# aokomoriuta/ConjugateGradient

Hardware: AMD Instinct MI355X
Metric: CG iterations/sec (7-pt Poisson 512^3); SpMV achieved HBM GB/s in roofline (higher is better)
Workload: dtype f64

## Files before the change

### conjugategradient_amd/csrc/common.hpp

```cpp
#pragma once
#include <hip/hip_runtime.h>
#include <cstddef>
#include <cstdint>
#include <cstdio>
#include <cstdarg>
#include <cstring>
#include <cmath>
#include <atomic>
#include <mutex>
#include <string>
#include <type_traits>
#include <vector>

#pragma GCC visibility push(default)
#include "../../include/MgcgGpu.h"
#pragma GCC visibility pop

namespace mgcg {

constexpr int kWave = 64;
constexpr int kBlock = 256;
constexpr int kNumXcd = 8;
constexpr int kNumCu = 256;
constexpr int kMaxGrid = kNumCu * 8;
// ... 101 lines not shown
    double alphaPrev, betaPrev;
    int live[kShiftMaxK];
};
struct ShiftScalars {
    double sigma[kShiftMaxK];
    ShiftState st[2];
    double residual[kShiftMaxK];
    int iteration[kShiftMaxK], status[kShiftMaxK];
};

struct MixedScalars {
    double maxrr, fMaxrr;
    int want, fWant;
    int gate;
    int updates;
    int fBroken;
    int pad;
};

struct SreduceScalars {
    double red[3];
    struct State { double gamma, alpha; } st[2];
};

struct MinresScalars {
    double red[5];
    int fDone, pad;
    struct State { double beta, cs, sn, dbar, eps, phibar, oldb; } st[2];
};

struct BlockScalars;
struct BkScalars;
struct Workspace {
    int device = -1;
    hipStream_t stream = nullptr;
    double* partials = nullptr;
    CgScalars* scalars = nullptr;
    HostMirror* mirror = nullptr;
    double* hostScalar = nullptr;
    int* devInts = nullptr;
    double* trace = nullptr;
    int traceCap = 0;
    double* ring[kXDeferMax] = {};
    long long ringSize = 0;
    double* blockPartials = nullptr;
    BlockScalars* blockScalars = nullptr;
    ShiftScalars* shiftScalars = nullptr;
    double* gramPartials = nullptr;
    BkScalars* bkScalars = nullptr;
    MixedScalars* mixedScalars = nullptr;
    float* mixedVecs = nullptr;
    long long mixedStride = 0;
    SreduceScalars* sreduceScalars = nullptr;
    MinresScalars* minresScalars = nullptr;
    bool init();
    void destroy();
    bool ensure_trace(int cap);
    bool ensure_ring(int slots, long long n);
    void free_ring();
    bool ensure_block();
    bool ensure_shift();
    bool ensure_bkrylov();
    bool ensure_mixed(long long n);
    bool ensure_sreduce();
    bool ensure_minres();
};

}

struct MgcgBlas   { mgcg::Workspace ws; };
namespace mgcg {
struct DcsrView {
    const unsigned char* colCode;
    const unsigned char* valCode;
    const int* deltaDict;
    const double* valueDict;
    int nDelta, nValue;
    long long rowBase;
    const unsigned char* patternId;
    const int* patCount;
    const int* patDelta;
    const double* patValue;
    int nPattern, patWidth;
    const double* tileVals;
    const int* tileCols;
    const int* tileRowIds;
    const int* tileStartHost;
    const unsigned* tilePacked;
    const int2* tileHdr;
    const int* tileHdrBaseHost;
    int tileShift;
    int tileWidth;
    int nTiles;
    long long tileRows;
    const double* pbVals;
    const unsigned short* pbCols;
    const unsigned short* pbPos;
    double* pbProd;
    const unsigned* pbPiece;
    const int* pbTileStart;
    const unsigned* pbPieceOff;
    const int* pbRoundOff;
    const unsigned short* pbRowBounds;
    int pbTiles, pbBlocks;
    long long pbColumns;
};
struct DcsrMatrix {
    const double* elements = nullptr; const int* rowOffsets = nullptr; const int* columnIndeces = nullptr;
    long long rows = 0, nnz = 0, rowBase = 0;
    unsigned char* colCode = nullptr; unsigned char* valCode = nullptr;
    int* deltaDict = nullptr; double* valueDict = nullptr;
    int nDelta = 0, nValue = 0;
    unsigned char* patternId = nullptr; int* patCount = nullptr; int* patDelta = nullptr; double* patValue = nullptr;
    int nPattern = 0, patWidth = 0;
    double* tileVals = nullptr; int* tileCols = nullptr; int* tileRowIds = nullptr; int nTiles = 0; long long tileRows = 0;
    unsigned* tilePacked = nullptr; int2* tileHdr = nullptr; int tileShift = 0, tileWidth = 0;
    std::vector<int> tileStart, tileHdrBase;
    double* pbVals = nullptr; unsigned short* pbCols = nullptr; unsigned short* pbPos = nullptr; double* pbProd = nullptr; unsigned* pbPiece = nullptr;
    unsigned* pbPieceOff = nullptr; int* pbTileStart = nullptr; int* pbRoundOff = nullptr; unsigned short* pbRowBounds = nullptr;
    int pbTiles = 0, pbBlocks = 0, pbMaxRounds = 0; long long pbColumns = 0;
    unsigned long long checksum = 0;
    int trustedUses = 0;
    bool automatic = false;
    bool usable = false;
    std::atomic<bool> stale{false};
    void release();
    DcsrView view() const
    {
        DcsrView v; v.colCode = colCode; v.valCode = valCode; v.deltaDict = deltaDict; v.valueDict = valueDict; v.nDelta = nDelta; v.nValue = nValue; v.rowBase = rowBase;
        v.patternId = patternId; v.patCount = patCount; v.patDelta = patDelta; v.patValue = patValue; v.nPattern = nPattern; v.patWidth = patWidth;
        v.tileVals = tileVals; v.tileCols = tileCols; v.tileRowIds = tileRowIds; v.tileStartHost = tileStart.data(); v.nTiles = nTiles; v.tileRows = tileRows;
        v.tilePacked = tilePacked; v.tileHdr = tileHdr; v.tileHdrBaseHost = tileHdrBase.data(); v.tileShift = tileShift; v.tileWidth = tileWidth;
        v.pbVals = pbVals; v.pbCols = pbCols; v.pbPos = pbPos; v.pbProd = pbProd; v.pbPiece = pbPiece; v.pbTileStart = pbTileStart; v.pbRoundOff = pbRoundOff;
        v.pbPieceOff = pbPieceOff; v.pbRowBounds = pbRowBounds; v.pbTiles = pbTiles; v.pbBlocks = pbBlocks; v.pbColumns = pbColumns;
        return v;
    }
};
struct SpmvProfile {
    bool enabled = false;
    std::vector<hipEvent_t> start, stop;
    int used = 0;
};
}
struct MgcgSparse {
    mgcg::Workspace ws;
    mgcg::SpmvProfile prof;
    int kernel = 0;
    int rowsPerBlock = 64;
    int flags = 0;
    int gridBlocks = 0;
    int periodRows = 0;
    int tileRows = 0, tilePlanes = 0;
    int analysedMode = 0;
    int compression = 0;
    std::vector<mgcg::DcsrMatrix*> analysed;
    struct PeriodEntry { const int* rowOffsets; const int* columnIndeces; long long rows, rowBase; int period; int maxRow; long long meanDistance;
                         int products = 0, threshold = 8; };
    std::vector<PeriodEntry> periods;
};
struct MgcgMatDescr { int type = 0; int base = 0; };
struct Vector    { double* data = nullptr; long long size = 0; int device = -1;
                   bool rawExported = false;
                   bool placed = false;
                   int drawCount = 0, drawChosen = -1; float drawMs[16] = {}; };
struct VectorInt { int* data = nullptr;    long long size = 0; int device = -1; };

namespace mgcg {

enum SpmvEpilogue {
    EPI_AXPBY = 0,
    EPI_DOT = 1,
    EPI_RESIDUAL = 2,
    EPI_JACOBI = 3,
    EPI_RESIDUAL_DOT = 4,
    EPI_AXPBY_BETA = 5,
    EPI_JACOBI_DOT = 6,
    EPI_CHEBYSHEV = 7,
    EPI_CHEBYSHEV_DOT = 8
};
#ifdef MGCG_LAB
#define MGCG_ABLATE(a, bits) (((a).ablate & (bits)) != 0)
#else
#define MGCG_ABLATE(a, bits) false
#endif
constexpr bool epi_has_dot(int e) { return e == EPI_DOT || e == EPI_RESIDUAL_DOT || e == EPI_JACOBI_DOT || e == EPI_CHEBYSHEV_DOT; }
constexpr bool epi_is_jacobi(int e) { return e == EPI_JACOBI || e == EPI_JACOBI_DOT; }
constexpr bool epi_is_chebyshev(int e) { return e == EPI_CHEBYSHEV || e == EPI_CHEBYSHEV_DOT; }

struct SpmvArgs {
    const double* elements;
    const int* rowOffsets;
    const int* columnIndeces;
    const double* x;
    double* y;
    int elementsCount;
    int rowCount;
    int columnCount;
    double alpha, beta;
    const double* w;
    const double* b;
    const double* dinv;
    double omega;
    int dinvUniform;
    double dinvScalar;
    double* d;
    double c1, c2;
    int xScaled;
    double xInner, xOuter;
    const double* xCoarse;
    int cM0, cM1, cM2, cS1, cS2;
    int cRowBase;
    double* partials;
    const int* doneFlag;
// ... 262 lines not shown
```

### conjugategradient_amd/csrc/kernels_dcsr.hip

```cpp
#include "common.hpp"
#include <algorithm>
#include <climits>

namespace mgcg {

typedef double d2 __attribute__((ext_vector_type(2)));
typedef unsigned u2 __attribute__((ext_vector_type(2)));

constexpr int kHashCap = 1024;
constexpr int kDictMax = 256;
constexpr int kEmptyDelta = INT_MIN;
constexpr unsigned long long kEmptyValue = 0xFFF8DEADBEEF0001ull;

__device__ inline void set_insert_delta(int* set, int* count, int key)
{
    unsigned h = ((unsigned)key * 2654435761u) & (kHashCap - 1);
    for (int probe = 0; probe < kHashCap; ++probe) {
        const int cur = set[h];
        if (cur == key) return;
        if (cur == kEmptyDelta) {
            const int prev = atomicCAS(&set[h], kEmptyDelta, key);
            if (prev == kEmptyDelta) { atomicAdd(count, 1); return; }
            if (prev == key) return;
        }
// ... 70 lines not shown
    h ^= h >> 33;
    return h;
}

__global__ __launch_bounds__(kBlock) void pattern_hash_kernel(const double* __restrict__ elements, const int* __restrict__ rowOffsets,
                                                              const int* __restrict__ columnIndeces, long long rows, long long rowBase,
                                                              unsigned long long* __restrict__ rowHash, unsigned long long* set, int* stats)
{
    const long long stride = (long long)gridDim.x * kBlock;
    int longest = 0;
    for (long long i = (long long)blockIdx.x * kBlock + threadIdx.x; i < rows; i += stride) {
        if (stats[0] > kPatMax) break;
        const int s = rowOffsets[i], e = rowOffsets[i + 1];
        unsigned long long h = pat_mix(0x243F6A8885A308D3ull, (unsigned long long)(e - s));
        for (int k = s; k < e; ++k) {
            h = pat_mix(h, (unsigned long long)((long long)columnIndeces[k] - (rowBase + i)));
            h = pat_mix(h, (unsigned long long)__double_as_longlong(elements[k]));
        }
        if (h == kPatEmpty) h = 1ull;
        rowHash[i] = h;
        longest = (e - s) > longest ? (e - s) : longest;
        unsigned slot = (unsigned)(h >> 20) & (kPatHashCap - 1);
        for (int probe = 0; probe < kPatHashCap; ++probe) {
            const unsigned long long cur = set[slot];
            if (cur == h) break;
            if (cur == kPatEmpty) {
                const unsigned long long prev = atomicCAS(&set[slot], kPatEmpty, h);
                if (prev == kPatEmpty) { atomicAdd(&stats[0], 1); break; }
                if (prev == h) break;
            }
            slot = (slot + 1) & (kPatHashCap - 1);
        }
    }
    atomicMax(&stats[1], longest);
}

__global__ __launch_bounds__(kBlock) void pattern_assign_kernel(const unsigned long long* __restrict__ rowHash, long long rows,
                                                                const unsigned long long* __restrict__ sorted, int n,
                                                                unsigned char* __restrict__ patternId, long long* rep)
{
    const long long stride = (long long)gridDim.x * kBlock;
    for (long long i = (long long)blockIdx.x * kBlock + threadIdx.x; i < rows; i += stride) {
        const int id = find_sorted(sorted, n, rowHash[i]);
        patternId[i] = (unsigned char)id;
        if (rep[id] > i) atomicMin((unsigned long long*)&rep[id], (unsigned long long)i);
    }
}

__global__ void pattern_table_kernel(const double* __restrict__ elements, const int* __restrict__ rowOffsets, const int* __restrict__ columnIndeces,
                                     long long rowBase, const long long* __restrict__ rep, int n, int width,
                                     int* __restrict__ patCount, int* __restrict__ patDelta, double* __restrict__ patValue)
{
    const int id = blockIdx.x * blockDim.x + threadIdx.x;
    if (id >= n) return;
    const long long i = rep[id];
    const int s = rowOffsets[i], e = rowOffsets[i + 1];
    patCount[id] = e - s;
    for (int j = 0; j < width; ++j) {
        const bool in = s + j < e;
        patDelta[id * width + j] = in ? (int)((long long)columnIndeces[s + j] - (rowBase + i)) : 0;
        patValue[id * width + j] = in ? elements[s + j] : 0.0;
    }
}

__global__ __launch_bounds__(kBlock) void pattern_verify_kernel(const double* __restrict__ elements, const int* __restrict__ rowOffsets,
                                                                const int* __restrict__ columnIndeces, long long rows, long long rowBase,
                                                                const unsigned char* __restrict__ patternId, int width,
                                                                const int* __restrict__ patCount, const int* __restrict__ patDelta,
                                                                const double* __restrict__ patValue, int* err)
{
    const long long stride = (long long)gridDim.x * kBlock;
    bool bad = false;
    for (long long i = (long long)blockIdx.x * kBlock + threadIdx.x; i < rows; i += stride) {
        const int id = patternId[i];
        const int s = rowOffsets[i], e = rowOffsets[i + 1];
        if (e - s != patCount[id]) { bad = true; continue; }
        for (int k = s; k < e; ++k) {
            const int d = (int)((long long)columnIndeces[k] - (rowBase + i));
            bad = bad || d != patDelta[id * width + (k - s)] ||
                  __double_as_longlong(elements[k]) != __double_as_longlong(patValue[id * width + (k - s)]);
        }
    }
    if (bad) atomicExch(err, 1);
}

void DcsrMatrix::release()
{
    if (colCode) (void)hipFree(colCode);
    if (valCode) (void)hipFree(valCode);
    if (deltaDict) (void)hipFree(deltaDict);
    if (valueDict) (void)hipFree(valueDict);
    if (patternId) (void)hipFree(patternId);
    if (patCount) (void)hipFree(patCount);
    if (patDelta) (void)hipFree(patDelta);
    if (patValue) (void)hipFree(patValue);
    if (tileVals) (void)hipFree(tileVals);
    if (tileCols) (void)hipFree(tileCols);
    if (tileRowIds) (void)hipFree(tileRowIds);
    if (tilePacked) (void)hipFree(tilePacked);
    if (tileHdr) (void)hipFree(tileHdr);
    tileVals = nullptr; tileCols = nullptr; tileRowIds = nullptr; nTiles = 0; tileRows = 0; tileStart.clear();
    tilePacked = nullptr; tileHdr = nullptr; tileShift = 0; tileWidth = 0; tileHdrBase.clear(); checksum = 0;
    for (void* p : { (void*)pbVals, (void*)pbCols, (void*)pbPos, (void*)pbProd, (void*)pbPiece, (void*)pbTileStart, (void*)pbPieceOff, (void*)pbRoundOff, (void*)pbRowBounds })
        if (p) (void)hipFree(p);
    pbVals = nullptr; pbCols = nullptr; pbPos = nullptr; pbProd = nullptr; pbPiece = nullptr; pbTileStart = nullptr; pbRoundOff = nullptr; pbPieceOff = nullptr;
    pbRowBounds = nullptr; pbTiles = pbBlocks = pbMaxRounds = 0; pbColumns = 0;
    colCode = valCode = nullptr; deltaDict = nullptr; valueDict = nullptr; nDelta = nValue = 0;
    patternId = nullptr; patCount = nullptr; patDelta = nullptr; patValue = nullptr; nPattern = patWidth = 0;
    usable = false;
}

bool pattern_build(hipStream_t s, const double* elements, const int* rowOffsets, const int* columnIndeces,
                   long long rows, long long nnz, long long rowBase, DcsrMatrix* out)
{
    if (rows <= 0 || nnz <= 0) return true;
    unsigned long long *rowHash = nullptr, *set = nullptr, *dSorted = nullptr;
    long long* rep = nullptr;
    int* stats = nullptr;
    unsigned char* ids = nullptr; int* pc = nullptr; int* pd = nullptr; double* pv = nullptr;
    auto cleanup = [&](bool keep) {
        for (void* p : { (void*)rowHash, (void*)set, (void*)dSorted, (void*)rep, (void*)stats }) if (p) (void)hipFree(p);
        if (!keep) for (void* p : { (void*)ids, (void*)pc, (void*)pd, (void*)pv }) if (p) (void)hipFree(p);
    };
    bool ok = MGCG_HIP(hipMalloc((void**)&rowHash, sizeof(unsigned long long) * (size_t)rows)) &&
              MGCG_HIP(hipMalloc((void**)&set, sizeof(unsigned long long) * kPatHashCap)) && MGCG_HIP(hipMalloc((void**)&stats, 3 * sizeof(int)));
    ok = ok && MGCG_HIP(hipMemsetAsync(set, 0, sizeof(unsigned long long) * kPatHashCap, s)) && MGCG_HIP(hipMemsetAsync(stats, 0, 3 * sizeof(int), s));
    if (!ok) { cleanup(false); return false; }
    long long blocks = (rows + kBlock - 1) / kBlock;
    if (blocks > kMaxGrid) blocks = kMaxGrid;
    hipLaunchKernelGGL(pattern_hash_kernel, dim3((int)blocks), dim3(kBlock), 0, s, elements, rowOffsets, columnIndeces, rows, rowBase, rowHash, set, stats);
    int hS[3] = { 0, 0, 0 };
    std::vector<unsigned long long> hSet(kPatHashCap);
    ok = MGCG_HIP(hipMemcpyAsync(hS, stats, sizeof(hS), hipMemcpyDeviceToHost, s)) &&
         MGCG_HIP(hipMemcpyAsync(hSet.data(), set, sizeof(unsigned long long) * kPatHashCap, hipMemcpyDeviceToHost, s)) && MGCG_HIP(hipStreamSynchronize(s));
    if (!ok) { cleanup(false); return false; }
    const int n = hS[0], width = hS[1];
    if (n < 1 || n > kPatMax || width < 1 || (long long)n * width > kPatEntries) { cleanup(false); return true; }
    std::vector<unsigned long long> sorted;
    for (unsigned long long v : hSet) if (v != kPatEmpty) sorted.push_back(v);
    std::sort(sorted.begin(), sorted.end());
    if ((int)sorted.size() != n) { cleanup(false); return true; }
    std::vector<long long> hRep((size_t)n, 0x7fffffffffffffffLL);
    ok = MGCG_HIP(hipMalloc((void**)&dSorted, sizeof(unsigned long long) * (size_t)n)) && MGCG_HIP(hipMalloc((void**)&rep, sizeof(long long) * (size_t)n)) &&
         MGCG_HIP(hipMalloc((void**)&ids, (size_t)rows + 16)) && MGCG_HIP(hipMalloc((void**)&pc, sizeof(int) * (size_t)n)) &&
         MGCG_HIP(hipMalloc((void**)&pd, sizeof(int) * (size_t)n * width)) && MGCG_HIP(hipMalloc((void**)&pv, sizeof(double) * (size_t)n * width));
    ok = ok && MGCG_HIP(hipMemcpyAsync(dSorted, sorted.data(), sizeof(unsigned long long) * (size_t)n, hipMemcpyHostToDevice, s)) &&
         MGCG_HIP(hipMemcpyAsync(rep, hRep.data(), sizeof(long long) * (size_t)n, hipMemcpyHostToDevice, s));
    if (!ok) { cleanup(false); return false; }
    hipLaunchKernelGGL(pattern_assign_kernel, dim3((int)blocks), dim3(kBlock), 0, s, rowHash, rows, dSorted, n, ids, rep);
    hipLaunchKernelGGL(pattern_table_kernel, dim3((n + 63) / 64), dim3(64), 0, s, elements, rowOffsets, columnIndeces, rowBase, rep, n, width, pc, pd, pv);
    hipLaunchKernelGGL(pattern_verify_kernel, dim3((int)blocks), dim3(kBlock), 0, s, elements, rowOffsets, columnIndeces, rows, rowBase, ids, width, pc, pd, pv, &stats[2]);
    ok = MGCG_HIP(hipGetLastError()) && MGCG_HIP(hipMemcpyAsync(hS, stats, sizeof(hS), hipMemcpyDeviceToHost, s)) && MGCG_HIP(hipStreamSynchronize(s));
    if (!ok) { cleanup(false); return false; }
    if (hS[2] != 0) { cleanup(false); return true; }
    out->patternId = ids; out->patCount = pc; out->patDelta = pd; out->patValue = pv; out->nPattern = n; out->patWidth = width;
    cleanup(true);
    return true;
}

bool dcsr_build(hipStream_t s, const double* elements, const int* rowOffsets, const int* columnIndeces,
                long long rows, long long nnz, long long rowBase, DcsrMatrix* out)
{
    out->release();
    out->elements = elements; out->rowOffsets = rowOffsets; out->columnIndeces = columnIndeces; out->rows = rows; out->nnz = nnz; out->rowBase = rowBase;
    if (rows <= 0 || nnz < 8) return true;
    int* dSet = nullptr; unsigned long long* vSet = nullptr; int* counts = nullptr;
    bool ok = MGCG_HIP(hipMalloc((void**)&dSet, sizeof(int) * kHashCap)) && MGCG_HIP(hipMalloc((void**)&vSet, sizeof(unsigned long long) * kHashCap)) &&
              MGCG_HIP(hipMalloc((void**)&counts, 2 * sizeof(int)));
    std::vector<int> hD(kHashCap, kEmptyDelta);
    std::vector<unsigned long long> hV(kHashCap, kEmptyValue);
    int hC[2] = { 0, 0 };
    ok = ok && MGCG_HIP(hipMemcpyAsync(dSet, hD.data(), sizeof(int) * kHashCap, hipMemcpyHostToDevice, s));
    ok = ok && MGCG_HIP(hipMemcpyAsync(vSet, hV.data(), sizeof(unsigned long long) * kHashCap, hipMemcpyHostToDevice, s));
    ok = ok && MGCG_HIP(hipMemcpyAsync(counts, hC, sizeof(hC), hipMemcpyHostToDevice, s));
    if (ok) {
        long long blocks = (rows + kBlock - 1) / kBlock;
        if (blocks > kMaxGrid) blocks = kMaxGrid;
        hipLaunchKernelGGL(dcsr_collect_kernel, dim3((int)blocks), dim3(kBlock), 0, s, elements, rowOffsets, columnIndeces, rows, rowBase, dSet, vSet, counts);
        ok = MGCG_HIP(hipMemcpyAsync(hC, counts, sizeof(hC), hipMemcpyDeviceToHost, s));
        ok = ok && MGCG_HIP(hipMemcpyAsync(hD.data(), dSet, sizeof(int) * kHashCap, hipMemcpyDeviceToHost, s));
        ok = ok && MGCG_HIP(hipMemcpyAsync(hV.data(), vSet, sizeof(unsigned long long) * kHashCap, hipMemcpyDeviceToHost, s));
        ok = ok && MGCG_HIP(hipStreamSynchronize(s));
    }
    if (dSet) (void)hipFree(dSet);
    if (vSet) (void)hipFree(vSet);
    if (counts) (void)hipFree(counts);
    if (!ok) return false;
    if (hC[0] > kDictMax) return true;
    std::vector<int> deltas;
    for (int v : hD) if (v != kEmptyDelta) deltas.push_back(v);
    std::sort(deltas.begin(), deltas.end());
    std::vector<unsigned long long> values;
    const bool val8 = hC[1] <= kDictMax;
    if (val8) { for (unsigned long long v : hV) if (v != kEmptyValue) values.push_back(v); std::sort(values.begin(), values.end()); }
    if ((int)deltas.size() != hC[0] || (val8 && (int)values.size() != hC[1])) { set_error("dcsr_build: inconsistent dictionary"); return false; }

    unsigned long long* dValBits = nullptr;
    ok = MGCG_HIP(hipMalloc((void**)&out->deltaDict, sizeof(int) * kDictMax)) && MGCG_HIP(hipMalloc((void**)&out->colCode, (size_t)nnz + 16));
    ok = ok && MGCG_HIP(hipMemcpyAsync(out->deltaDict, deltas.data(), sizeof(int) * deltas.size(), hipMemcpyHostToDevice, s));
    if (val8) {
        ok = ok && MGCG_HIP(hipMalloc((void**)&out->valueDict, sizeof(double) * kDictMax)) && MGCG_HIP(hipMalloc((void**)&out->valCode, (size_t)nnz + 16));
        ok = ok && MGCG_HIP(hipMalloc((void**)&dValBits, sizeof(unsigned long long) * kDictMax));
        ok = ok && MGCG_HIP(hipMemcpyAsync(dValBits, values.data(), sizeof(unsigned long long) * values.size(), hipMemcpyHostToDevice, s));
        ok = ok && MGCG_HIP(hipMemcpyAsync(out->valueDict, values.data(), sizeof(double) * values.size(), hipMemcpyHostToDevice, s));
    }
    if (ok) {
        long long blocks = (rows + kBlock - 1) / kBlock;
        if (blocks > kMaxGrid) blocks = kMaxGrid;
        hipLaunchKernelGGL(dcsr_encode_kernel, dim3((int)blocks), dim3(kBlock), 0, s, elements, rowOffsets, columnIndeces, rows, rowBase,
                           out->deltaDict, (int)deltas.size(), dValBits, (int)values.size(), out->colCode, val8 ? out->valCode : nullptr);
        ok = MGCG_HIP(hipGetLastError()) && MGCG_HIP(hipStreamSynchronize(s));
    }
    if (dValBits) (void)hipFree(dValBits);
    if (!ok) { out->release(); return false; }
    out->nDelta = (int)deltas.size(); out->nValue = (int)values.size(); out->usable = true;
    return true;
}

void preload_kernels_dcsr() { preload_code_object(reinterpret_cast<const void*>(&dcsr_collect_kernel)); }

}
```

### conjugategradient_amd/csrc/kernels_rows.hip

```cpp
#include "common.hpp"
#include "spmv_epilogue.hpp"

namespace mgcg {

typedef double d2 __attribute__((ext_vector_type(2)));
typedef int i2 __attribute__((ext_vector_type(2)));
typedef unsigned u2 __attribute__((ext_vector_type(2)));

enum { FMT_CSR = 0, FMT_DCSR8 = 1, FMT_DCSR64 = 2 };

constexpr int kRR = 64;
constexpr int kRCap = 512;
constexpr int kRAlign = 32;
constexpr int kRDict = 256;

template <int FMT>
struct RowsStage {
    i2 col[4];
    d2 val[4];
    u2 cc, vc;
    int my_s, my_e;
    int s, e;
};

// ... 108 lines not shown
            __syncthreads();
            double acc = 0.0;
            int k = cur.my_s;
            const int passEnd0 = tb0 + kRCap;
            double xg[8], vv[8];
            int cnt = cur.my_e - k; cnt = cnt < 8 ? cnt : 8;
            { const int room = passEnd0 - k; cnt = cnt < room ? cnt : room; cnt = cnt > 0 ? cnt : 0; }
#pragma unroll
            for (int j = 0; j < 8; ++j) {
                int idx = k + j - tb0;
                idx = (j < cnt) ? idx : 0;
                long long col;
                if constexpr (FMT == FMT_CSR) { col = s_col[idx]; vv[j] = s_val[idx]; }
                else {
                    col = myRowGlobal + s_dD[s_cc[idx]];
                    if constexpr (FMT == FMT_DCSR8) vv[j] = s_vD[s_vc[idx]]; else vv[j] = s_val[idx];
                }
                if (j >= cnt) col = 0;
                if (MGCG_ABLATE(a, 2)) col &= 1023;
                xg[j] = a.x[col];
            }
            long long myRow = r0 + tid;
            myRow = myRow <= lastRow ? myRow : lastRow;
            const RowsEpi eo = rows_epi_prefetch<EPI>(a, myRow);
            issue(nxt, t + 1 < nTrips ? rb_of(t + 1) : rb);
            if (pendRow >= 0 && !MGCG_ABLATE(a, 1)) a.y[pendRow] = pendVal;
#pragma unroll
            for (int j = 0; j < 8; ++j) { const double p = vv[j] * xg[j]; acc += (j < cnt) ? p : 0.0; }
            k += cnt;
            int tb = tb0;
            while (true) {
                const int passEnd = tb + kRCap;
                const int stop = cur.my_e < passEnd ? cur.my_e : passEnd;
                for (; k < stop; ++k) {
                    const int idx = k - tb;
                    long long col; double v;
                    if constexpr (FMT == FMT_CSR) { col = s_col[idx]; v = s_val[idx]; }
                    else { col = myRowGlobal + s_dD[s_cc[idx]]; if constexpr (FMT == FMT_DCSR8) v = s_vD[s_vc[idx]]; else v = s_val[idx]; }
                    const double p = v * a.x[col];
                    acc += p;
                }
                tb += kRCap;
                if (tb >= e) break;
                __syncthreads();
                RowsStage<FMT> more;
                more.s = cur.s; more.e = cur.e; more.my_s = cur.my_s; more.my_e = cur.my_e;
                load_pass(more, tb);
                stage_pass(more, tb, e);
                __syncthreads();
            }
            pendRow = -1;
            if (tid < nr) { pendVal = rows_epilogue_value<EPI>(a, acc, eo, dotacc); pendRow = r0 + tid; }
            if (MGCG_ABLATE(a, 1) && acc == 1.2345e300) pendRow = 0;
            __syncthreads();
            cur = nxt;
            nxt.s = s2; nxt.e = e2;
        }
        if (pendRow >= 0 && !MGCG_ABLATE(a, 1)) a.y[pendRow] = pendVal;
    }
    if constexpr (epi_has_dot(EPI)) {
        double v = dotacc;
#pragma unroll
        for (int off = 32; off > 0; off >>= 1) v += __shfl_down(v, off, 64);
        if (tid == 0) a.partials[blockIdx.x] = v;
    }
}

template <int EPI>
static int launch_rows_epi(hipStream_t s, const SpmvArgs& a, const DcsrView* m, int gridReq)
{
    const int nRowBlocks = (int)(((long long)a.rowCount + kRR - 1) / kRR);
    DeviceState* d = device_state();
    int grid = gridReq > 0 ? gridReq : (m == nullptr ? 8 : 16) * (d ? d->numCu : kNumCu);
    if (grid > kMaxPartials) grid = kMaxPartials;
    if (grid > nRowBlocks) grid = nRowBlocks;
    if (grid < 1) grid = 1;
    DcsrView none{};
    if (m == nullptr) hipLaunchKernelGGL((spmv_rows_kernel<EPI, FMT_CSR>), dim3(grid), dim3(64), 0, s, a, none, nRowBlocks);
    else if (m->valCode != nullptr) hipLaunchKernelGGL((spmv_rows_kernel<EPI, FMT_DCSR8>), dim3(grid), dim3(64), 0, s, a, *m, nRowBlocks);
    else hipLaunchKernelGGL((spmv_rows_kernel<EPI, FMT_DCSR64>), dim3(grid), dim3(64), 0, s, a, *m, nRowBlocks);
    return grid;
}

template <int EPI, int CH>
__global__ __launch_bounds__(64) void spmv_pattern_kernel(SpmvArgs a, DcsrView m, int nRowBlocks, int groupBlocks, TileMap tm)
{
    constexpr int RPL = 2;
    extern __shared__ __attribute__((aligned(16))) unsigned char s_raw[];
    const int W = m.patWidth, nP = m.nPattern;
    double* s_val = (double*)s_raw;
    int* s_delta = (int*)(s_val + nP * W);
    int* s_cnt = s_delta + nP * W;
    if (a.doneFlag != nullptr && *a.doneFlag != 0) return;
    const int tid = threadIdx.x;
    for (int i = tid; i < nP * W; i += 64) { s_val[i] = m.patValue[i]; s_delta[i] = m.patDelta[i]; }
    for (int i = tid; i < nP; i += 64) s_cnt[i] = m.patCount[i];
    __syncthreads();

    const bool grouped = groupBlocks > 0 && (gridDim.x & 7) == 0;
    const long long G = grouped ? groupBlocks : 1;
    const int xcd = grouped ? (int)(blockIdx.x & 7) : 0;
    const long long first = grouped ? (long long)(blockIdx.x >> 3) : (long long)blockIdx.x;
    const long long step = grouped ? (long long)(gridDim.x >> 3) : (long long)gridDim.x;
    const long long count = grouped ? (((long long)nRowBlocks + 8 * G - 1) / (8 * G)) * G : (long long)nRowBlocks;
    auto block_of = [&](long long L) -> long long { return grouped ? ((L / G) * 8 + xcd) * G + (L % G) : L; };

    const long long lastRow = (long long)a.rowCount - 1;
    auto load_ids = [&](long long rb, int* pid) {
        const long long base = rb * (64 * RPL);
#pragma unroll
        for (int u = 0; u < RPL; ++u) { long long r = base + u * 64 + tid; r = r <= lastRow ? r : lastRow; r = r >= 0 ? r : 0; pid[u] = m.patternId[r]; }
    };
    const bool sweep = tm.mode != 0;
    const long long nTrips = sweep ? tile_map_trips(tm, (int)blockIdx.x, (int)gridDim.x, nRowBlocks) : (count > first ? (count - first + step - 1) / step : 0);
    auto trip_block = [&](long long t) -> long long { return sweep ? (long long)tile_map_tile(tm, (int)t, (int)blockIdx.x, (int)gridDim.x) : block_of(first + t * step); };
    double dotacc = 0.0;
    int pidNext[RPL];
    if (nTrips > 0) load_ids(trip_block(0) < nRowBlocks ? trip_block(0) : 0, pidNext);
    for (long long t = 0; t < nTrips; ++t) {
        const long long rb = trip_block(t);
        int pid[RPL];
#pragma unroll
        for (int u = 0; u < RPL; ++u) pid[u] = pidNext[u];
        if (t + 1 < nTrips) { const long long nb = trip_block(t + 1); load_ids(nb < nRowBlocks ? nb : 0, pidNext); }
        if (rb >= nRowBlocks) continue;
        const long long base = rb * (64 * RPL);
        long long row[RPL]; bool live[RPL]; int tb[RPL], cnt[RPL]; double acc[RPL]; RowsEpi eo[RPL];
#pragma unroll
        for (int u = 0; u < RPL; ++u) {
            row[u] = base + u * 64 + tid;
            live[u] = row[u] <= lastRow;
            row[u] = live[u] ? row[u] : lastRow;
        }
#pragma unroll
        for (int u = 0; u < RPL; ++u) { eo[u] = rows_epi_prefetch<EPI>(a, row[u]); tb[u] = pid[u] * W; cnt[u] = s_cnt[pid[u]]; acc[u] = 0.0; }
        int longest = 0, shortest = 0x7fffffff;
#pragma unroll
        for (int u = 0; u < RPL; ++u) { longest = cnt[u] > longest ? cnt[u] : longest; shortest = cnt[u] < shortest ? cnt[u] : shortest; }
#pragma unroll
        for (int off = 32; off > 0; off >>= 1) {
            const int o = __shfl_xor(longest, off, 64), q = __shfl_xor(shortest, off, 64);
            longest = o > longest ? o : longest; shortest = q < shortest ? q : shortest;
        }
        if (shortest == CH && longest == CH) {
            double xg[RPL][CH], vv[RPL][CH];
#pragma unroll
            for (int u = 0; u < RPL; ++u) {
                const long long g = m.rowBase + row[u];
#pragma unroll
                for (int j = 0; j < CH; ++j) {
                    vv[u][j] = s_val[tb[u] + j];
                    long long col = g + s_delta[tb[u] + j];
                    if (MGCG_ABLATE(a, 2)) col &= 1023;
                    xg[u][j] = a.x[col];
                }
            }
            if (a.xScaled) {
#pragma unroll
                for (int u = 0; u < RPL; ++u)
#pragma unroll
                    for (int j = 0; j < CH; ++j) { const double t = a.xInner * xg[u][j]; xg[u][j] = a.xOuter * t; }
            }
#pragma unroll
            for (int u = 0; u < RPL; ++u)
#pragma unroll
                for (int j = 0; j < CH; ++j) { const double p = vv[u][j] * xg[u][j]; acc[u] += p; }
        } else {
            for (int j0 = 0; j0 < longest; j0 += CH) {
                double xg[RPL][CH], vv[RPL][CH];
#pragma unroll
                for (int u = 0; u < RPL; ++u) {
                    const long long g = m.rowBase + row[u];
#pragma unroll
                    for (int j = 0; j < CH; ++j) {
                        const bool on = j0 + j < cnt[u];
                        const int t = tb[u] + (on ? j0 + j : 0);
                        vv[u][j] = s_val[t];
                        xg[u][j] = a.x[g + s_delta[t]];
                    }
                }
                if (a.xScaled) {
#pragma unroll
                    for (int u = 0; u < RPL; ++u)
#pragma unroll
                        for (int j = 0; j < CH; ++j) { const double t = a.xInner * xg[u][j]; xg[u][j] = a.xOuter * t; }
                }
#pragma unroll
                for (int u = 0; u < RPL; ++u)
#pragma unroll
                    for (int j = 0; j < CH; ++j) { const double p = vv[u][j] * xg[u][j]; acc[u] += (j0 + j < cnt[u]) ? p : 0.0; }
            }
        }
#pragma unroll
        for (int u = 0; u < RPL; ++u)
            if (live[u]) {
                const double v = rows_epilogue_value<EPI>(a, acc[u], eo[u], dotacc);
                if (!MGCG_ABLATE(a, 1) || v == 1.2345e300) a.y[row[u]] = v;
            }
    }
    if constexpr (epi_has_dot(EPI)) {
        double v = dotacc;
#pragma unroll
        for (int off = 32; off > 0; off >>= 1) v += __shfl_down(v, off, 64);
        if (tid == 0) a.partials[blockIdx.x] = v;
    }
}

constexpr int kPatternWavesPerCu = 16;

template <int EPI>
static int launch_pattern_epi(hipStream_t s, const SpmvArgs& a, const DcsrView& m, int gridReq, int periodRows)
{
    const int nRowBlocks = (int)(((long long)a.rowCount + 127) / 128);
    DeviceState* d = device_state();
    int grid = gridReq > 0 ? gridReq : kPatternWavesPerCu * (d ? d->numCu : kNumCu);
    if (grid > kMaxPartials) grid = kMaxPartials;
    if (grid > nRowBlocks) grid = nRowBlocks;
    if (grid < 1) grid = 1;
    const size_t lds = (size_t)m.nPattern * m.patWidth * 12 + (size_t)m.nPattern * 4;
    const int group = 0;
    TileMap tm = make_tile_map(a.rowCount, (a.rowCount % 128 != 0) ? 0 : periodRows, grid, 128);
    if (m.patWidth == 7) hipLaunchKernelGGL((spmv_pattern_kernel<EPI, 7>), dim3(grid), dim3(64), lds, s, a, m, nRowBlocks, group, tm);
    else if (m.patWidth == 5) hipLaunchKernelGGL((spmv_pattern_kernel<EPI, 5>), dim3(grid), dim3(64), lds, s, a, m, nRowBlocks, group, tm);
    else hipLaunchKernelGGL((spmv_pattern_kernel<EPI, 8>), dim3(grid), dim3(64), lds, s, a, m, nRowBlocks, group, tm);
    return grid;
}

static int launch_spmv_pattern(hipStream_t s, int epilogue, const SpmvArgs& a, const DcsrView& m, int gridReq, int periodRows)
{
    switch (epilogue) {
    case EPI_AXPBY:        return a.beta != 0.0 ? launch_pattern_epi<EPI_AXPBY_BETA>(s, a, m, gridReq, periodRows) : launch_pattern_epi<EPI_AXPBY>(s, a, m, gridReq, periodRows);
    case EPI_DOT:          return launch_pattern_epi<EPI_DOT>(s, a, m, gridReq, periodRows);
    case EPI_RESIDUAL:     return launch_pattern_epi<EPI_RESIDUAL>(s, a, m, gridReq, periodRows);
    case EPI_RESIDUAL_DOT: return launch_pattern_epi<EPI_RESIDUAL_DOT>(s, a, m, gridReq, periodRows);
    case EPI_JACOBI:       return launch_pattern_epi<EPI_JACOBI>(s, a, m, gridReq, periodRows);
    case EPI_JACOBI_DOT:   return launch_pattern_epi<EPI_JACOBI_DOT>(s, a, m, gridReq, periodRows);
    }
    return 0;
}

int launch_spmv_rows(hipStream_t s, int epilogue, const SpmvArgs& a, const DcsrView* m, int gridReq, int periodRows)
{
    if (a.rowCount <= 0) return 0;
    if (m != nullptr && m->patternId != nullptr) return launch_spmv_pattern(s, epilogue, a, *m, gridReq, periodRows);
    switch (epilogue) {
    case EPI_AXPBY:        return a.beta != 0.0 ? launch_rows_epi<EPI_AXPBY_BETA>(s, a, m, gridReq) : launch_rows_epi<EPI_AXPBY>(s, a, m, gridReq);
    case EPI_DOT:          return launch_rows_epi<EPI_DOT>(s, a, m, gridReq);
    case EPI_RESIDUAL:     return launch_rows_epi<EPI_RESIDUAL>(s, a, m, gridReq);
    case EPI_RESIDUAL_DOT: return launch_rows_epi<EPI_RESIDUAL_DOT>(s, a, m, gridReq);
    case EPI_JACOBI:       return launch_rows_epi<EPI_JACOBI>(s, a, m, gridReq);
    case EPI_JACOBI_DOT:   return launch_rows_epi<EPI_JACOBI_DOT>(s, a, m, gridReq);
    case EPI_CHEBYSHEV:    return launch_rows_epi<EPI_CHEBYSHEV>(s, a, m, gridReq);
    case EPI_CHEBYSHEV_DOT: return launch_rows_epi<EPI_CHEBYSHEV_DOT>(s, a, m, gridReq);
    }
    return 0;
}

void preload_kernels_rows() { preload_code_object(reinterpret_cast<const void*>(&(spmv_rows_kernel<EPI_DOT, FMT_CSR>))); }

}
```

Measured before the change: 270.4.

## Add dominant-pattern fast path with wave-uniform stencil loads in pattern SpMV

Setup now builds a histogram of row pattern IDs and records the dominant full-width pattern as a reference. The SpMV kernel holds that pattern's coefficients and offsets in scalar registers and, for rows using it, loads x through a scalar base plus a lane offset, avoiding per-lane LDS lookups and 64-bit address arithmetic. Other rows take a per-lane general path. The kernel also changes from 64-thread blocks handling two rows per lane to 256-thread workgroups of four waves, one row per lane, with a different tile map and grid sizing. This trades per-row indirection for more divergence when patterns are mixed, plus extra histogram work at setup.

```diff
diff --git a/conjugategradient_amd/csrc/common.hpp b/conjugategradient_amd/csrc/common.hpp
--- a/conjugategradient_amd/csrc/common.hpp
+++ b/conjugategradient_amd/csrc/common.hpp
@@ -207,6 +207,7 @@
     const int* patDelta;
     const double* patValue;
     int nPattern, patWidth;
+    int refPattern;
     const double* tileVals;
     const int* tileCols;
     const int* tileRowIds;
@@ -237,7 +238,7 @@
     int* deltaDict = nullptr; double* valueDict = nullptr;
     int nDelta = 0, nValue = 0;
     unsigned char* patternId = nullptr; int* patCount = nullptr; int* patDelta = nullptr; double* patValue = nullptr;
-    int nPattern = 0, patWidth = 0;
+    int nPattern = 0, patWidth = 0, refPattern = -1;
     double* tileVals = nullptr; int* tileCols = nullptr; int* tileRowIds = nullptr; int nTiles = 0; long long tileRows = 0;
     unsigned* tilePacked = nullptr; int2* tileHdr = nullptr; int tileShift = 0, tileWidth = 0;
     std::vector<int> tileStart, tileHdrBase;
@@ -253,7 +254,7 @@
     DcsrView view() const
     {
         DcsrView v; v.colCode = colCode; v.valCode = valCode; v.deltaDict = deltaDict; v.valueDict = valueDict; v.nDelta = nDelta; v.nValue = nValue; v.rowBase = rowBase;
-        v.patternId = patternId; v.patCount = patCount; v.patDelta = patDelta; v.patValue = patValue; v.nPattern = nPattern; v.patWidth = patWidth;
+        v.patternId = patternId; v.patCount = patCount; v.patDelta = patDelta; v.patValue = patValue; v.nPattern = nPattern; v.patWidth = patWidth; v.refPattern = refPattern;
         v.tileVals = tileVals; v.tileCols = tileCols; v.tileRowIds = tileRowIds; v.tileStartHost = tileStart.data(); v.nTiles = nTiles; v.tileRows = tileRows;
         v.tilePacked = tilePacked; v.tileHdr = tileHdr; v.tileHdrBaseHost = tileHdrBase.data(); v.tileShift = tileShift; v.tileWidth = tileWidth;
         v.pbVals = pbVals; v.pbCols = pbCols; v.pbPos = pbPos; v.pbProd = pbProd; v.pbPiece = pbPiece; v.pbTileStart = pbTileStart; v.pbRoundOff = pbRoundOff;
diff --git a/conjugategradient_amd/csrc/kernels_dcsr.hip b/conjugategradient_amd/csrc/kernels_dcsr.hip
--- a/conjugategradient_amd/csrc/kernels_dcsr.hip
+++ b/conjugategradient_amd/csrc/kernels_dcsr.hip
@@ -176,6 +176,26 @@
         }
     }
     if (bad) atomicExch(err, 1);
+}
+
+__global__ __launch_bounds__(kBlock) void pattern_histogram_kernel(const unsigned char* __restrict__ patternId, long long rows, unsigned long long* hist)
+{
+    __shared__ unsigned int s_hist[kPatMax];
+    for (int i = threadIdx.x; i < kPatMax; i += kBlock) s_hist[i] = 0u;
+    __syncthreads();
+    const long long stride = (long long)gridDim.x * kBlock;
+    for (long long i = (long long)blockIdx.x * kBlock + threadIdx.x; i < rows; i += stride) atomicAdd(&s_hist[patternId[i]], 1u);
+    __syncthreads();
+    for (int i = threadIdx.x; i < kPatMax; i += kBlock)
+        if (s_hist[i] != 0u) atomicAdd(&hist[i], (unsigned long long)s_hist[i]);
+}
+
+__global__ void pattern_dominant_kernel(const unsigned long long* __restrict__ hist, int n, int width, const int* __restrict__ patCount, int* ref)
+{
+    if (blockIdx.x != 0 || threadIdx.x != 0) return;
+    int best = 0;
+    for (int id = 1; id < n; ++id) if (hist[id] > hist[best]) best = id;
+    *ref = patCount[best] == width ? best : -1;
 }
 
 void DcsrMatrix::release()
@@ -200,7 +220,7 @@
     pbVals = nullptr; pbCols = nullptr; pbPos = nullptr; pbProd = nullptr; pbPiece = nullptr; pbTileStart = nullptr; pbRoundOff = nullptr; pbPieceOff = nullptr;
     pbRowBounds = nullptr; pbTiles = pbBlocks = pbMaxRounds = 0; pbColumns = 0;
     colCode = valCode = nullptr; deltaDict = nullptr; valueDict = nullptr; nDelta = nValue = 0;
-    patternId = nullptr; patCount = nullptr; patDelta = nullptr; patValue = nullptr; nPattern = patWidth = 0;
+    patternId = nullptr; patCount = nullptr; patDelta = nullptr; patValue = nullptr; nPattern = patWidth = 0; refPattern = -1;
     usable = false;
 }
 
@@ -208,12 +228,12 @@
                    long long rows, long long nnz, long long rowBase, DcsrMatrix* out)
 {
     if (rows <= 0 || nnz <= 0) return true;
-    unsigned long long *rowHash = nullptr, *set = nullptr, *dSorted = nullptr;
+    unsigned long long *rowHash = nullptr, *set = nullptr, *dSorted = nullptr, *hist = nullptr;
     long long* rep = nullptr;
     int* stats = nullptr;
     unsigned char* ids = nullptr; int* pc = nullptr; int* pd = nullptr; double* pv = nullptr;
     auto cleanup = [&](bool keep) {
-        for (void* p : { (void*)rowHash, (void*)set, (void*)dSorted, (void*)rep, (void*)stats }) if (p) (void)hipFree(p);
+        for (void* p : { (void*)rowHash, (void*)set, (void*)dSorted, (void*)hist, (void*)rep, (void*)stats }) if (p) (void)hipFree(p);
         if (!keep) for (void* p : { (void*)ids, (void*)pc, (void*)pd, (void*)pv }) if (p) (void)hipFree(p);
     };
     bool ok = MGCG_HIP(hipMalloc((void**)&rowHash, sizeof(unsigned long long) * (size_t)rows)) &&
@@ -247,6 +267,15 @@
     ok = MGCG_HIP(hipGetLastError()) && MGCG_HIP(hipMemcpyAsync(hS, stats, sizeof(hS), hipMemcpyDeviceToHost, s)) && MGCG_HIP(hipStreamSynchronize(s));
     if (!ok) { cleanup(false); return false; }
     if (hS[2] != 0) { cleanup(false); return true; }
+    int ref = -1;
+    ok = MGCG_HIP(hipMalloc((void**)&hist, sizeof(unsigned long long) * kPatMax)) && MGCG_HIP(hipMemsetAsync(hist, 0, sizeof(unsigned long long) * kPatMax, s));
+    if (ok) {
+        hipLaunchKernelGGL(pattern_histogram_kernel, dim3((int)blocks), dim3(kBlock), 0, s, ids, rows, hist);
+        hipLaunchKernelGGL(pattern_dominant_kernel, dim3(1), dim3(64), 0, s, hist, n, width, pc, &stats[0]);
+        ok = MGCG_HIP(hipGetLastError()) && MGCG_HIP(hipMemcpyAsync(&ref, &stats[0], sizeof(int), hipMemcpyDeviceToHost, s)) && MGCG_HIP(hipStreamSynchronize(s));
+    }
+    if (!ok) { cleanup(false); return false; }
+    out->refPattern = (ref >= 0 && ref < n) ? ref : -1;
     out->patternId = ids; out->patCount = pc; out->patDelta = pd; out->patValue = pv; out->nPattern = n; out->patWidth = width;
     cleanup(true);
     return true;
diff --git a/conjugategradient_amd/csrc/kernels_rows.hip b/conjugategradient_amd/csrc/kernels_rows.hip
--- a/conjugategradient_amd/csrc/kernels_rows.hip
+++ b/conjugategradient_amd/csrc/kernels_rows.hip
@@ -214,148 +214,158 @@
     return grid;
 }
 
+constexpr int kPW = 4;
+constexpr int kPTileRows = 64 * kPW;
+constexpr int kPatternWgPerCu = 2;
+constexpr int kPatternTripTiles = 1;
+constexpr bool kPatternNtStore = false;
+
+__device__ __forceinline__ double pattern_uniform(double v)
+{
+    const int lo = __builtin_amdgcn_readfirstlane(__double2loint(v)), hi = __builtin_amdgcn_readfirstlane(__double2hiint(v));
+    return __hiloint2double(hi, lo);
+}
+
+typedef const __attribute__((address_space(1))) char* pattern_gptr;
+
 template <int EPI, int CH>
-__global__ __launch_bounds__(64) void spmv_pattern_kernel(SpmvArgs a, DcsrView m, int nRowBlocks, int groupBlocks, TileMap tm)
-{
-    constexpr int RPL = 2;
+__global__ __launch_bounds__(64 * kPW) void spmv_pattern_kernel(SpmvArgs a, DcsrView m, int nRowBlocks, int nTiles, TileMap tm)
+{
+    constexpr int U = kPatternTripTiles;
     extern __shared__ __attribute__((aligned(16))) unsigned char s_raw[];
     const int W = m.patWidth, nP = m.nPattern;
     double* s_val = (double*)s_raw;
     int* s_delta = (int*)(s_val + nP * W);
     int* s_cnt = s_delta + nP * W;
     if (a.doneFlag != nullptr && *a.doneFlag != 0) return;
-    const int tid = threadIdx.x;
-    for (int i = tid; i < nP * W; i += 64) { s_val[i] = m.patValue[i]; s_delta[i] = m.patDelta[i]; }
-    for (int i = tid; i < nP; i += 64) s_cnt[i] = m.patCount[i];
+    const int tid = threadIdx.x & 63;
+    const int wv = __builtin_amdgcn_readfirstlane((int)(threadIdx.x >> 6));
+    for (int i = threadIdx.x; i < nP * W; i += 64 * kPW) { s_val[i] = m.patValue[i]; s_delta[i] = m.patDelta[i]; }
+    for (int i = threadIdx.x; i < nP; i += 64 * kPW) s_cnt[i] = m.patCount[i];
     __syncthreads();
 
-    const bool grouped = groupBlocks > 0 && (gridDim.x & 7) == 0;
-    const long long G = grouped ? groupBlocks : 1;
-    const int xcd = grouped ? (int)(blockIdx.x & 7) : 0;
-    const long long first = grouped ? (long long)(blockIdx.x >> 3) : (long long)blockIdx.x;
-    const long long step = grouped ? (long long)(gridDim.x >> 3) : (long long)gridDim.x;
-    const long long count = grouped ? (((long long)nRowBlocks + 8 * G - 1) / (8 * G)) * G : (long long)nRowBlocks;
-    auto block_of = [&](long long L) -> long long { return grouped ? ((L / G) * 8 + xcd) * G + (L % G) : L; };
+    const int ref = W <= CH ? m.refPattern : -1;
+    const int nF = W;
+    double rv[CH]; int rd[CH];
+#pragma unroll
+    for (int j = 0; j < CH; ++j) {
+        const int e = (ref >= 0 && j < nF) ? ref * W + j : 0;
+        rv[j] = pattern_uniform(s_val[e]);
+        rd[j] = __builtin_amdgcn_readfirstlane(s_delta[e]);
+    }
 
     const long long lastRow = (long long)a.rowCount - 1;
-    auto load_ids = [&](long long rb, int* pid) {
-        const long long base = rb * (64 * RPL);
-#pragma unroll
-        for (int u = 0; u < RPL; ++u) { long long r = base + u * 64 + tid; r = r <= lastRow ? r : lastRow; r = r >= 0 ? r : 0; pid[u] = m.patternId[r]; }
-    };
-    const bool sweep = tm.mode != 0;
-    const long long nTrips = sweep ? tile_map_trips(tm, (int)blockIdx.x, (int)gridDim.x, nRowBlocks) : (count > first ? (count - first + step - 1) / step : 0);
-    auto trip_block = [&](long long t) -> long long { return sweep ? (long long)tile_map_tile(tm, (int)t, (int)blockIdx.x, (int)gridDim.x) : block_of(first + t * step); };
+    const int wg = blockIdx.x, nWG = gridDim.x;
+    const int nTrips = tile_map_trips(tm, wg, nWG, nTiles);
+    auto block_of = [&](int t) -> long long { return (long long)tile_map_tile(tm, t, wg, nWG) * kPW + wv; };
+    auto load_id = [&](long long rb) -> int { long long r = rb * 64 + tid; r = r <= lastRow ? r : lastRow; return m.patternId[r]; };
     double dotacc = 0.0;
-    int pidNext[RPL];
-    if (nTrips > 0) load_ids(trip_block(0) < nRowBlocks ? trip_block(0) : 0, pidNext);
-    for (long long t = 0; t < nTrips; ++t) {
-        const long long rb = trip_block(t);
-        int pid[RPL];
-#pragma unroll
-        for (int u = 0; u < RPL; ++u) pid[u] = pidNext[u];
-        if (t + 1 < nTrips) { const long long nb = trip_block(t + 1); load_ids(nb < nRowBlocks ? nb : 0, pidNext); }
-        if (rb >= nRowBlocks) continue;
-        const long long base = rb * (64 * RPL);
-        long long row[RPL]; bool live[RPL]; int tb[RPL], cnt[RPL]; double acc[RPL]; RowsEpi eo[RPL];
-#pragma unroll
-        for (int u = 0; u < RPL; ++u) {
-            row[u] = base + u * 64 + tid;
-            live[u] = row[u] <= lastRow;
-            row[u] = live[u] ? row[u] : lastRow;
-        }
-#pragma unroll
-        for (int u = 0; u < RPL; ++u) { eo[u] = rows_epi_prefetch<EPI>(a, row[u]); tb[u] = pid[u] * W; cnt[u] = s_cnt[pid[u]]; acc[u] = 0.0; }
-        int longest = 0, shortest = 0x7fffffff;
-#pragma unroll
-        for (int u = 0; u < RPL; ++u) { longest = cnt[u] > longest ? cnt[u] : longest; shortest = cnt[u] < shortest ? cnt[u] : shortest; }
-#pragma unroll
-        for (int off = 32; off > 0; off >>= 1) {
-            const int o = __shfl_xor(longest, off, 64), q = __shfl_xor(shortest, off, 64);
-            longest = o > longest ? o : longest; shortest = q < shortest ? q : shortest;
-        }
-        if (shortest == CH && longest == CH) {
-            double xg[RPL][CH], vv[RPL][CH];
-#pragma unroll
-            for (int u = 0; u < RPL; ++u) {
+    int pidNext[U];
+#pragma unroll
+    for (int u = 0; u < U; ++u) pidNext[u] = u < nTrips ? load_id(block_of(u)) : 0;
+    for (int t0 = 0; t0 < nTrips; t0 += U) {
+        int pid[U]; long long rb[U]; bool on[U];
+#pragma unroll
+        for (int u = 0; u < U; ++u) {
+            pid[u] = pidNext[u];
+            on[u] = t0 + u < nTrips;
+            rb[u] = on[u] ? block_of(t0 + u) : 0;
+            on[u] = on[u] && rb[u] < nRowBlocks;
+        }
+#pragma unroll
+        for (int u = 0; u < U; ++u)
+            if (t0 + U + u < nTrips) pidNext[u] = load_id(block_of(t0 + U + u));
+        long long row[U]; bool live[U], fastLane[U]; double acc[U]; RowsEpi eo[U]; double xg[U][CH];
+#pragma unroll
+        for (int u = 0; u < U; ++u) {
+            row[u] = rb[u] * 64 + tid;
+            live[u] = on[u] && row[u] <= lastRow;
+            row[u] = row[u] <= lastRow ? row[u] : lastRow;
+            fastLane[u] = live[u] && pid[u] == ref;
+            eo[u] = rows_epi_prefetch<EPI>(a, row[u]);
+            acc[u] = 0.0;
+        }
+#pragma unroll
+        for (int u = 0; u < U; ++u)
+            if (fastLane[u]) {
+                const double* xb = a.x + (m.rowBase + rb[u] * 64);
+                unsigned lane8 = (unsigned)tid << 3;
+                asm volatile("" : "+v"(lane8));
+#pragma unroll
+                for (int j = 0; j < CH; ++j)
+                    if (CH != 8 || j < nF) {
+                        pattern_gptr sb = (pattern_gptr)(MGCG_ABLATE(a, 2) ? a.x + j : xb + rd[j]);
+                        asm volatile("" : "+s"(sb));
+                        xg[u][j] = *(const __attribute__((address_space(1))) double*)(sb + lane8);
+                    }
+            }
+#pragma unroll
+        for (int u = 0; u < U; ++u)
+            if (live[u] && !fastLane[u]) {
                 const long long g = m.rowBase + row[u];
-#pragma unroll
-                for (int j = 0; j < CH; ++j) {
-                    vv[u][j] = s_val[tb[u] + j];
-                    long long col = g + s_delta[tb[u] + j];
-                    if (MGCG_ABLATE(a, 2)) col &= 1023;
-                    xg[u][j] = a.x[col];
-                }
-            }
-            if (a.xScaled) {
-#pragma unroll
-                for (int u = 0; u < RPL; ++u)
-#pragma unroll
-                    for (int j = 0; j < CH; ++j) { const double t = a.xInner * xg[u][j]; xg[u][j] = a.xOuter * t; }
-            }
-#pragma unroll
-            for (int u = 0; u < RPL; ++u)
-#pragma unroll
-                for (int j = 0; j < CH; ++j) { const double p = vv[u][j] * xg[u][j]; acc[u] += p; }
-        } else {
-            for (int j0 = 0; j0 < longest; j0 += CH) {
-                double xg[RPL][CH], vv[RPL][CH];
-#pragma unroll
-                for (int u = 0; u < RPL; ++u) {
-                    const long long g = m.rowBase + row[u];
+                const int tb = pid[u] * W, cnt = s_cnt[pid[u]];
+                for (int j0 = 0; j0 < cnt; j0 += CH) {
+                    double xo[CH], vv[CH];
 #pragma unroll
                     for (int j = 0; j < CH; ++j) {
-                        const bool on = j0 + j < cnt[u];
-                        const int t = tb[u] + (on ? j0 + j : 0);
-                        vv[u][j] = s_val[t];
-                        xg[u][j] = a.x[g + s_delta[t]];
+                        const bool in = j0 + j < cnt;
+                        const int t = tb + (in ? j0 + j : 0);
+                        vv[j] = s_val[t];
+                        xo[j] = a.x[g + s_delta[t]];
                     }
-                }
+                    if (a.xScaled) {
+#pragma unroll
+                        for (int j = 0; j < CH; ++j) { const double t = a.xInner * xo[j]; xo[j] = a.xOuter * t; }
+                    }
+#pragma unroll
+                    for (int j = 0; j < CH; ++j) { const double p = vv[j] * xo[j]; acc[u] += (j0 + j < cnt) ? p : 0.0; }
+                }
+            }
+#pragma unroll
+        for (int u = 0; u < U; ++u)
+            if (fastLane[u]) {
                 if (a.xScaled) {
 #pragma unroll
-                    for (int u = 0; u < RPL; ++u)
-#pragma unroll
-                        for (int j = 0; j < CH; ++j) { const double t = a.xInner * xg[u][j]; xg[u][j] = a.xOuter * t; }
-                }
-#pragma unroll
-                for (int u = 0; u < RPL; ++u)
-#pragma unroll
-                    for (int j = 0; j < CH; ++j) { const double p = vv[u][j] * xg[u][j]; acc[u] += (j0 + j < cnt[u]) ? p : 0.0; }
-            }
-        }
-#pragma unroll
-        for (int u = 0; u < RPL; ++u)
+                    for (int j = 0; j < CH; ++j)
+                        if (CH != 8 || j < nF) { const double t = a.xInner * xg[u][j]; xg[u][j] = a.xOuter * t; }
+                }
+#pragma unroll
+                for (int j = 0; j < CH; ++j)
+                    if (CH != 8 || j < nF) { const double p = rv[j] * xg[u][j]; acc[u] += p; }
+            }
+#pragma unroll
+        for (int u = 0; u < U; ++u)
             if (live[u]) {
                 const double v = rows_epilogue_value<EPI>(a, acc[u], eo[u], dotacc);
-                if (!MGCG_ABLATE(a, 1) || v == 1.2345e300) a.y[row[u]] = v;
+                if (!MGCG_ABLATE(a, 1) || v == 1.2345e300) {
+                    if constexpr (kPatternNtStore) __builtin_nontemporal_store(v, a.y + row[u]); else a.y[row[u]] = v;
+                }
             }
     }
     if constexpr (epi_has_dot(EPI)) {
         double v = dotacc;
 #pragma unroll
         for (int off = 32; off > 0; off >>= 1) v += __shfl_down(v, off, 64);
-        if (tid == 0) a.partials[blockIdx.x] = v;
-    }
-}
-
-constexpr int kPatternWavesPerCu = 16;
+        if (tid == 0) a.partials[blockIdx.x * kPW + wv] = v;
+    }
+}
 
 template <int EPI>
 static int launch_pattern_epi(hipStream_t s, const SpmvArgs& a, const DcsrView& m, int gridReq, int periodRows)
 {
-    const int nRowBlocks = (int)(((long long)a.rowCount + 127) / 128);
+    const int nRowBlocks = (int)(((long long)a.rowCount + 63) / 64);
+    const int nTiles = (int)(((long long)a.rowCount + kPTileRows - 1) / kPTileRows);
     DeviceState* d = device_state();
-    int grid = gridReq > 0 ? gridReq : kPatternWavesPerCu * (d ? d->numCu : kNumCu);
-    if (grid > kMaxPartials) grid = kMaxPartials;
-    if (grid > nRowBlocks) grid = nRowBlocks;
-    if (grid < 1) grid = 1;
+    int nWG = gridReq > 0 ? gridReq / kPW : kPatternWgPerCu * (d ? d->numCu : kNumCu);
+    if (nWG * kPW > kMaxPartials) nWG = kMaxPartials / kPW;
+    if (nWG > nTiles) nWG = nTiles;
+    if (nWG < 1) nWG = 1;
     const size_t lds = (size_t)m.nPattern * m.patWidth * 12 + (size_t)m.nPattern * 4;
-    const int group = 0;
-    TileMap tm = make_tile_map(a.rowCount, (a.rowCount % 128 != 0) ? 0 : periodRows, grid, 128);
-    if (m.patWidth == 7) hipLaunchKernelGGL((spmv_pattern_kernel<EPI, 7>), dim3(grid), dim3(64), lds, s, a, m, nRowBlocks, group, tm);
-    else if (m.patWidth == 5) hipLaunchKernelGGL((spmv_pattern_kernel<EPI, 5>), dim3(grid), dim3(64), lds, s, a, m, nRowBlocks, group, tm);
-    else hipLaunchKernelGGL((spmv_pattern_kernel<EPI, 8>), dim3(grid), dim3(64), lds, s, a, m, nRowBlocks, group, tm);
-    return grid;
+    TileMap tm = make_tile_map(a.rowCount, periodRows, nWG, kPTileRows);
+    if (m.patWidth == 7) hipLaunchKernelGGL((spmv_pattern_kernel<EPI, 7>), dim3(nWG), dim3(64 * kPW), lds, s, a, m, nRowBlocks, nTiles, tm);
+    else if (m.patWidth == 5) hipLaunchKernelGGL((spmv_pattern_kernel<EPI, 5>), dim3(nWG), dim3(64 * kPW), lds, s, a, m, nRowBlocks, nTiles, tm);
+    else hipLaunchKernelGGL((spmv_pattern_kernel<EPI, 8>), dim3(nWG), dim3(64 * kPW), lds, s, a, m, nRowBlocks, nTiles, tm);
+    return nWG * kPW;
 }
 
 static int launch_spmv_pattern(hipStream_t s, int epilogue, const SpmvArgs& a, const DcsrView& m, int gridReq, int periodRows)
```

After: 272.2 (median of 2 runs). About the same (+0.7%).
